# ClickHouse/libhdfs3

Hardware: AMD Instinct MI355X
Metric: device-resident CRC32C GiB/s over 512 B HDFS chunks; % of HBM roofline (higher is better)
Workload: dtype u8

## Files before the change

libhdfs3_amd/csrc/client/block_reader.cpp:

```cpp
#include "hdfs3_client.h"

#include <hip/hip_runtime.h>
#include <sys/socket.h>
#include <sys/uio.h>
#include <time.h>

#include <algorithm>
#include <cerrno>
#include <chrono>
#include <condition_variable>
#include <cstdlib>
#include <cstring>
#include <deque>
#include <mutex>
#include <new>
#include <string>
#include <thread>
#include <vector>

#include "../copy_pool.h"
#include "../ctx.h"
#include "../numa.h"
#include "block_reader.h"
#include "hdfs3_crc.h"
#include "net.h"
#include "wire.h"

using namespace hdfs3crc;

namespace {

constexpr int kDefaultBatchPackets = 64;
constexpr int kDefaultTimeoutMs = 60000;
constexpr size_t kMaxResponse = 10u << 20;
constexpr int kSlots = 3;
constexpr int kPhases = 8;
constexpr int kWaitPollUs = 20;
std::atomic<uint64_t> g_phase_ns[kPhases] = {};

uint64_t thread_cpu_ns() {
    timespec ts{};
    clock_gettime(CLOCK_THREAD_CPUTIME_ID, &ts);
    return uint64_t(ts.tv_sec) * 1000000000ull + uint64_t(ts.tv_nsec);
}
constexpr int kMaxSlots = 64;
constexpr int32_t kMaxPacketData = 16 << 20;
constexpr size_t kArenaCacheMax = 6;
constexpr size_t kPacketGuess = 64 * 1024 + 512 + 16;

struct PacketRef {
    uint64_t data_off, crc_off;
    uint32_t data_len;
    uint32_t skip;
    uint32_t deliver;
};

struct Batch {
    PacketArena a;
    size_t used = 0;
    std::vector<PacketRef> pk;
    bool verified = false;
    int64_t bad_pkt = -1;
    size_t dpkt = 0, doff = 0;
    bool dense = false, sealed = false;
    uint64_t d0 = 0, words_used = 0, data_used = 0;
    std::vector<uint64_t> chunk0;
    bool uploaded = false;

    void reset() {
        used = 0;
        pk.clear();
        verified = false;
        bad_pkt = -1;
        dpkt = doff = 0;
        dense = sealed = false;
        d0 = words_used = data_used = 0;
        chunk0.clear();
        uploaded = false;
    }
};

bool dense_bpc(uint32_t bpc) { return round_bpc(bpc) || pieces_bpc(bpc); }

bool wire_layout_forced() {
    static const bool f = [] {
        const char *e = getenv("HDFS3_READER_LAYOUT");
        return e && std::strcmp(e, "wire") == 0;
    }();
    return f;
}

uint64_t now_ns() {
    return uint64_t(std::chrono::duration_cast<std::chrono::nanoseconds>(
                        std::chrono::steady_clock::now().time_since_epoch()).count());
}

struct Timer {
    std::atomic<uint64_t> &acc;
    uint64_t t0 = now_ns();
    explicit Timer(std::atomic<uint64_t> &a) : acc(a) {}
    ~Timer() { acc.fetch_add(now_ns() - t0, std::memory_order_relaxed); }
};

thread_local bool t_hip_fault = false;

#if HDFS3_LAB
std::atomic<int> g_fail_prefetch_arenas{0};
#endif

int hip_err(hipError_t e, const char *what) {
    t_hip_fault = true;
    return fail(e == hipErrorOutOfMemory ? -ENOMEM : -EIO, "%s: %s", what, hipGetErrorString(e));
}

#define HIP_OK(expr)                                      \
    do {                                                  \
        hipError_t e_ = (expr);                           \
        if (e_ != hipSuccess) return hip_err(e_, #expr);  \
    } while (0)

int grow(PacketArena &a, size_t cap, size_t descs) {
    if (cap > a.cap) {
        if (a.h) (void)hipHostFree(a.h);
        if (a.d) (void)hipFree(a.d);
        a.h = a.d = nullptr;
        a.cap = 0;
        HIP_OK(hipHostMalloc(reinterpret_cast<void **>(&a.h), cap, pinned_host_flags()));
        HIP_OK(hipMalloc(reinterpret_cast<void **>(&a.d), cap));
        a.cap = cap;
    }
    if (descs > a.desc_cap) {
        if (a.h_desc) (void)hipHostFree(a.h_desc);
        if (a.d_desc) (void)hipFree(a.d_desc);
        a.h_desc = a.d_desc = nullptr;
        a.desc_cap = 0;
        HIP_OK(hipHostMalloc(reinterpret_cast<void **>(&a.h_desc), descs * sizeof(DevSegment), pinned_host_flags()));
        HIP_OK(hipMalloc(reinterpret_cast<void **>(&a.d_desc), descs * sizeof(DevSegment)));
        a.desc_cap = descs;
    }
    if (!a.d_res) {
        HIP_OK(hipMalloc(reinterpret_cast<void **>(&a.d_res), sizeof(unsigned long long)));
        HIP_OK(hipHostMalloc(reinterpret_cast<void **>(&a.h_res), sizeof(unsigned long long), pinned_host_flags()));
        HIP_OK(hipEventCreateWithFlags(&a.done, hipEventDisableTiming | hipEventBlockingSync));
    }
    return 0;
}

}

struct hdfs3_block_reader {
    int fd = -1;
    int timeout_ms = kDefaultTimeoutMs;
    int batch_packets = kDefaultBatchPackets;
    bool verify = true;
    hdfs3_crc_ctx *ctx = nullptr;
    bool own_ctx = true;
    bool prefetch = false;
    wire::ExtendedBlock block;
    int64_t start = 0, end_offset = 0;
    uint32_t chunk_size = 0;
    uint32_t checksum_size = 0;
    const uint32_t *tables = nullptr;

    int64_t recv_cursor = 0;
    int64_t last_seqno = -1;
    bool range_done = false;
    bool trailer_ok = false;
    std::atomic<bool> local_fault{false};
    bool have_pending_hdr = false;
    wire::PacketHeader pending_hdr;
    bool header_ahead = true;
    bool have_next_raw = false;
    uint8_t next_raw[wire::kPacketHeaderSize];

    std::mutex mu;
    std::condition_variable cv;
    std::vector<Batch> slot;
    std::deque<int> ready;
    std::deque<int> free_slots;
    bool recv_done = false;
    int recv_error = 0;
    std::string recv_msg;
    bool stop = false;
    std::thread rx;

    int64_t delivered = 0;
    bool sent_status = false;
    int error = 0;
    std::string error_msg;

    std::atomic<uint64_t> packets{0}, batches{0};
    std::atomic<uint64_t> dev_launches{0}, dev_bytes{0};
    hipEvent_t dev_done = nullptr;
    std::atomic<uint64_t> t_ns[kPhases] = {};
    enum WaitMode { kWaitPoll, kWaitBlock, kWaitSpin } wait_mode = kWaitPoll;
    bool copy_nt = false;
    uint8_t *dest = nullptr;
    int64_t rx_out = 0;
    void eager(const uint8_t *src, int64_t useful) {
        if (dest && useful > 0 && rx_out + useful <= end_offset - start) std::memcpy(dest + rx_out, src, size_t(useful));
        rx_out += useful;
    }

    int sticky(int code, const std::string &msg) {
        error = code;
        error_msg = msg;
        return fail(code, "%s", msg.c_str());
    }

    int check_response() {
        std::string resp;
        if (int rc = net::read_delimited(fd, resp, kMaxResponse, timeout_ms))
            return sticky(rc, "RemoteBlockReader: failed to read BlockOpResponseProto");
        wire::BlockOpResponse r;
        if (!wire::decode_block_op_response(resp.data(), resp.size(), r))
            return sticky(-EPROTO, "RemoteBlockReader cannot parse BlockOpResponseProto from Datanode response");
        if (r.status != wire::kSuccess)
            return sticky(-EIO, "RemoteBlockReader: Datanode return an error when sending read request: " +
                                    (r.message.empty() ? std::string("check Datanode's log") : r.message));
        if (!r.has_checksum_info) return sticky(-EPROTO, "RemoteBlockReader: response lacks ReadOpChecksumInfoProto");
        chunk_size = r.bytes_per_checksum;
        switch (r.checksum_type) {
        case wire::kChecksumNull: verify = false; checksum_size = 0; break;
        case wire::kChecksumCrc32c: checksum_size = 4; tables = ctx->d_tables_by[0]; break;
        case wire::kChecksumCrc32: checksum_size = 4; tables = ctx->d_tables_by[1]; break;
        default: return sticky(-EPROTO, "RemoteBlockReader cannot recognize checksum type");
        }
        if (chunk_size == 0 || chunk_size > 0x7FFFFFFFu)
            return sticky(-EPROTO, "RemoteBlockReader invalid chunk size");
        const int64_t first = int64_t(r.chunk_offset);
        if (first < 0 || first > start || first <= start - int64_t(chunk_size))
            return sticky(-EPROTO, "RemoteBlockReader invalid first chunk offset");
        return 0;
    }

    int rx_fail(int code, const std::string &msg) {
        recv_msg = msg;
        return code;
    }

    int read_header(wire::PacketHeader &h) {
        if (have_pending_hdr) {
            h = pending_hdr;
            have_pending_hdr = false;
            return 0;
        }
        if (have_next_raw) {
            have_next_raw = false;
            if (!h.decode(next_raw, sizeof(next_raw))) return rx_fail(-EPROTO, "Invalid PacketHeader");
            return 0;
        }
        uint8_t buf[wire::kPacketHeaderSize];
        if (int rc = net::recv_fully(fd, buf, sizeof(buf)))
            return rx_fail(rc, "RemoteBlockReader: failed to read block header");
        if (!h.decode(buf, sizeof(buf))) return rx_fail(-EPROTO, "Invalid PacketHeader");
        return 0;
    }

    int receive(Batch &b) {
        Timer tm(t_ns[0]);
        b.reset();
        while (int(b.pk.size()) < batch_packets && !range_done) {
            wire::PacketHeader h;
            if (int rc = read_header(h)) return rc;
            if (!h.sanity_check(last_seqno)) return rx_fail(-EIO, "RemoteBlockReader: Packet failed on sanity check");
            if (h.data_len <= 0) {
                last_seqno = h.seqno;
                range_done = true;
                break;
            }
            if (h.data_len > kMaxPacketData) return rx_fail(-EIO, "Invalid Packet, dataLen exceeds 16 MiB");
            if (h.offset_in_block > recv_cursor || recv_cursor - h.offset_in_block >= h.data_len)
                return rx_fail(-EIO, "Invalid Packet, offsetInBlock does not continue the block");
            const uint64_t chunks = (uint64_t(h.data_len) + chunk_size - 1) / chunk_size;
            const uint64_t crc_len = chunks * checksum_size;
            if (int64_t(h.packet_len) != 4 + int64_t(h.data_len) + int64_t(crc_len))
                return rx_fail(-EIO, "Invalid Packet, packetLen does not match dataLen and checksums");
            const uint64_t size = crc_len + uint64_t(h.data_len);
            if (b.pk.empty())
                b.dense = verify && checksum_size == 4 && dense_bpc(chunk_size) && !wire_layout_forced();
            if (b.dense) {
                if (b.pk.empty()) {
                    const uint64_t exp_data = std::max<uint64_t>(uint64_t(h.data_len), uint64_t(64) << 10);
                    const uint64_t max_crc = (exp_data + chunk_size - 1) / chunk_size * checksum_size;
                    b.d0 = (uint64_t(batch_packets) * max_crc + 4095) & ~uint64_t(4095);
                    const uint64_t need = b.d0 + uint64_t(h.data_len);
                    if (need > b.a.cap)
                        if (int rc = grow(b.a, need, size_t(batch_packets))) return rx_fail(rc, "arena growth failed");
                } else if (b.sealed || b.words_used + crc_len > b.d0 ||
                           b.d0 + b.data_used + uint64_t(h.data_len) > b.a.cap) {
                    pending_hdr = h;
                    have_pending_hdr = true;
                    break;
                }
                iovec v[3] = {{b.a.h + b.words_used, crc_len}, {b.a.h + b.d0 + b.data_used, size_t(h.data_len)},
                              {next_raw, header_ahead ? sizeof(next_raw) : 0}};
                if (int rc = net::recv_fully_iov(fd, v, 3))
                    return rx_fail(rc, "RemoteBlockReader: failed to read packet payload");
                have_next_raw = header_ahead;
                last_seqno = h.seqno;
                packets.fetch_add(1, std::memory_order_relaxed);
                int64_t ahead = recv_cursor - h.offset_in_block;
                ahead = ahead > 0 ? ahead : 0;
                const int64_t useful =
                    std::max<int64_t>(0, std::min<int64_t>(h.data_len - ahead, end_offset - recv_cursor));
                b.pk.push_back(PacketRef{b.d0 + b.data_used, b.words_used, uint32_t(h.data_len), uint32_t(ahead),
                                         uint32_t(useful)});
                eager(b.a.h + b.d0 + b.data_used + ahead, useful);
                b.chunk0.push_back(b.words_used / 4);
                b.words_used += crc_len;
                b.data_used += uint64_t(h.data_len);
                b.used = b.d0 + b.data_used;
                if (h.data_len % chunk_size) b.sealed = true;
                const int64_t reached = recv_cursor + h.data_len - ahead;
                recv_cursor = reached;
                if (reached >= end_offset) {
                    if (int rc = read_trailer()) return rc;
                    range_done = true;
                }
                continue;
            }
            uint64_t off = ((b.used + crc_len + 15) & ~uint64_t(15)) - crc_len;
            if (off + size > b.a.cap) {
                if (!b.pk.empty()) {
                    pending_hdr = h;
                    have_pending_hdr = true;
                    break;
                }
                if (int rc = grow(b.a, size + 64, size_t(batch_packets))) return rx_fail(rc, "arena growth failed");
                off = ((crc_len + 15) & ~uint64_t(15)) - crc_len;
            }
            iovec v[2] = {{b.a.h + off, size}, {next_raw, header_ahead ? sizeof(next_raw) : 0}};
            if (int rc = net::recv_fully_iov(fd, v, 2))
                return rx_fail(rc, "RemoteBlockReader: failed to read packet payload");
            have_next_raw = header_ahead;
            last_seqno = h.seqno;
            packets.fetch_add(1, std::memory_order_relaxed);
            int64_t ahead = recv_cursor - h.offset_in_block;
            ahead = ahead > 0 ? ahead : 0;
            const int64_t useful = std::max<int64_t>(0, std::min<int64_t>(h.data_len - ahead, end_offset - recv_cursor));
            b.pk.push_back(PacketRef{off + crc_len, off, uint32_t(h.data_len), uint32_t(ahead), uint32_t(useful)});
            eager(b.a.h + off + crc_len + ahead, useful);
            b.used = off + size;
            const int64_t reached = recv_cursor + h.data_len - ahead;
            recv_cursor = reached;
            if (reached >= end_offset) {
                if (int rc = read_trailer()) return rc;
                range_done = true;
            }
        }
        return 0;
    }

    int read_trailer() {
        wire::PacketHeader t;
        if (int rc = read_header(t)) return rc;
        if (t.last_packet_in_block && t.data_len == 0) {
            last_seqno = t.seqno;
            trailer_ok = true;
        }
        return 0;
    }

    int launch(Batch &b) {
        Timer tm(t_ns[2]);
        batches.fetch_add(1, std::memory_order_relaxed);
        if (!verify) {
            b.verified = true;
            return 0;
        }
        LaunchEnv env = launch_env(ctx, &b.a.pieces);
        env.tables = tables;
        env.fold = ctx->d_fold_by[tables == ctx->d_tables_by[1]];
        HIP_OK(hipMemcpyAsync(b.a.d, b.a.h, b.used, hipMemcpyHostToDevice, ctx->stream));
        b.uploaded = true;
        HIP_OK(hipMemsetAsync(b.a.d_res, 0, sizeof(unsigned long long), ctx->stream));
        if (b.dense) {
            ChunkLaunch a{};
            a.data = b.a.d + b.d0;
            a.len = b.data_used;
            a.bpc = chunk_size;
            a.crc_be = b.a.d;
            a.result = b.a.d_res;
            a.check_short_tail = 0;
            HIP_OK(launch_chunks(env, a, true));
        } else {
            std::vector<DevPacket> hp(b.pk.size());
            for (size_t i = 0; i < b.pk.size(); ++i)
                hp[i] = DevPacket{b.pk[i].data_off, b.pk[i].crc_off, b.pk[i].data_len, 0};
            HIP_OK(launch_packet_batch(env, b.a.d, hp.data(), hp.size(), chunk_size, true, 0,
                                       b.a.d_res, b.a.h_desc, b.a.d_desc));
        }
        ++ctx->launches;
        HIP_OK(hipMemcpyAsync(b.a.h_res, b.a.d_res, sizeof(unsigned long long), hipMemcpyDeviceToHost, ctx->stream));
        HIP_OK(hipEventRecord(b.a.done, ctx->stream));
        return 0;
    }

    int acquire(Batch &b) {
        Timer tm(t_ns[1]);
#if HDFS3_LAB
        if (prefetch && g_fail_prefetch_arenas.load() > 0 && g_fail_prefetch_arenas.fetch_sub(1) > 0) {
            t_hip_fault = true;
            return rx_fail(fail(-ENOMEM, "injected pinned-memory shortage"), "arena allocation failed");
        }
#endif
        if (!b.a.h) {
            std::lock_guard<std::mutex> lk(ctx->arena_mu);
            if (!ctx->arena_cache.empty()) {
                b.a = ctx->arena_cache.back();
                ctx->arena_cache.pop_back();
            }
        }
        if (int rc = grow(b.a, std::max(b.a.cap, size_t(batch_packets) * kPacketGuess), size_t(batch_packets)))
            return rx_fail(rc, "arena allocation failed");
        return 0;
    }

    void receiver() {
        (void)hipSetDevice(ctx->device);
        bind_thread_to_device(ctx->device);
        const uint64_t cpu0 = thread_cpu_ns();
        struct CpuAdd {
            hdfs3_block_reader *r;
            uint64_t c0;
            ~CpuAdd() { r->t_ns[7].fetch_add(thread_cpu_ns() - c0, std::memory_order_relaxed); }
        } cpu_add{this, cpu0};
        for (;;) {
            int s;
            {
                Timer idle(t_ns[5]);
                std::unique_lock<std::mutex> lk(mu);
                cv.wait(lk, [&] { return stop || !free_slots.empty(); });
                if (stop) break;
                s = free_slots.front();
                free_slots.pop_front();
            }
            Batch &b = slot[s];
            t_hip_fault = false;
            int rc = acquire(b);
            if (!rc) rc = receive(b);
            if (!rc && !b.pk.empty()) {
                rc = launch(b);
                if (rc) recv_msg = hdfs3_crc_last_error();
            }
            if (rc && t_hip_fault) local_fault = true;
            {
                std::lock_guard<std::mutex> lk(mu);
                if (!rc && !b.pk.empty())
                    ready.push_back(s);
                else
                    free_slots.push_back(s);
                if (rc) recv_error = rc;
                if (rc || range_done) recv_done = true;
            }
            cv.notify_all();
            if (rc || range_done) break;
        }
    }

    void start_receiver() {
        for (int i = 0; i < int(slot.size()); ++i) free_slots.push_back(i);
        rx = std::thread([this] { receiver(); });
    }

    int wait_event(hipEvent_t ev) {
        Timer tm(t_ns[3]);
        if (wait_mode == kWaitBlock) {
            HIP_OK(hipEventSynchronize(ev));
        } else {
            for (;;) {
                const hipError_t q = hipEventQuery(ev);
                if (q == hipSuccess) break;
                if (q != hipErrorNotReady) HIP_OK(q);
                if (wait_mode == kWaitPoll) std::this_thread::sleep_for(std::chrono::microseconds(kWaitPollUs));
            }
        }
        return 0;
    }

    int wait(Batch &b) {
        if (b.verified) return 0;
        if (int rc = wait_event(b.a.done)) return rc;
        const unsigned long long r = *b.a.h_res;
        if (r && b.dense) {
            const uint64_t chunk = ~r;
            b.bad_pkt = int64_t(std::upper_bound(b.chunk0.begin(), b.chunk0.end(), chunk) - b.chunk0.begin()) - 1;
        } else if (r) {
            b.bad_pkt = int64_t((~r) >> 32);
        }
        b.verified = true;
        return 0;
    }

    void maybe_send_status() {
        if (sent_status || error || !trailer_ok) return;
        {
            std::lock_guard<std::mutex> lk(mu);
            if (!recv_done || recv_error || !ready.empty()) return;
        }
        const std::string msg = wire::encode_client_read_status(verify ? wire::kChecksumOk : wire::kSuccess);
        if (net::write_delimited(fd, msg, timeout_ms) == 0) sent_status = true;
    }

    int32_t read(uint8_t *out, int32_t len) {
        if (error) return fail(error, "%s", error_msg.c_str());
        if (len <= 0 || !out) return fail(-EINVAL, "invalid read buffer");
        int32_t total = 0;
        while (total < len) {
            int s;
            {
                Timer idle(t_ns[6]);
                std::unique_lock<std::mutex> lk(mu);
                cv.wait(lk, [&] { return !ready.empty() || recv_done; });
                if (ready.empty()) {
                    if (recv_error) {
                        const int code = recv_error;
                        const std::string msg = recv_msg;
                        lk.unlock();
                        if (total) {
                            error = code;
                            error_msg = msg;
                            return total;
                        }
                        return sticky(code, msg);
                    }
                    break;
                }
                s = ready.front();
            }
            Batch &b = slot[s];
            if (int rc = wait(b)) {
                local_fault = true;
                return total ? total : sticky(rc, hdfs3_crc_last_error());
            }
            const size_t limit = b.bad_pkt >= 0 ? size_t(b.bad_pkt) : b.pk.size();
            {
                Timer tm(t_ns[4]);
                while (total < len && b.dpkt < limit) {
                    const PacketRef &p = b.pk[b.dpkt];
                    const size_t avail = p.deliver - b.doff;
                    const size_t n = std::min<size_t>(avail, size_t(len - total));
                    if (dest && out + total == dest + delivered)
                        ;
                    else if (copy_nt && n >= 4096)
                        memcpy_stream(out + total, b.a.h + p.data_off + p.skip + b.doff, n);
                    else
                        std::memcpy(out + total, b.a.h + p.data_off + p.skip + b.doff, n);
                    total += int32_t(n);
                    b.doff += n;
                    delivered += int64_t(n);
                    if (b.doff == p.deliver) {
                        ++b.dpkt;
                        b.doff = 0;
                    }
                }
            }
            if (b.dpkt == limit) {
                if (b.bad_pkt >= 0) {
                    sticky(-EIO, "ChecksumException: RemoteBlockReader: checksum not match for Block: " +
                                     std::to_string(block.block_id) + " (packet " + std::to_string(b.bad_pkt) +
                                     " of a GPU batch)");
                    return total ? total : error;
                }
                {
                    std::lock_guard<std::mutex> lk(mu);
                    ready.pop_front();
                    free_slots.push_back(s);
                }
                cv.notify_all();
            }
        }
        maybe_send_status();
        return total;
    }

    int32_t read_dev(uint8_t *d_out, int32_t len) {
        if (error) return fail(error, "%s", error_msg.c_str());
        if (len <= 0 || !d_out) return fail(-EINVAL, "invalid read buffer");
        DeviceGuard guard(ctx->device);
        hipPointerAttribute_t at{};
        if (hipPointerGetAttributes(&at, d_out) != hipSuccess || at.type != hipMemoryTypeDevice ||
            at.device != ctx->device) {
            (void)hipGetLastError();
            return fail(-EINVAL, "read_dev: the buffer is not device memory of device %d", ctx->device);
        }
        if (!dev_done) HIP_OK(hipEventCreateWithFlags(&dev_done, hipEventDisableTiming | hipEventBlockingSync));
        int32_t total = 0;
        int failed = 0;
        bool enqueued = false;
        std::vector<CopyRange> rg;
        auto complete = [&]() -> int {
            if (!enqueued) return 0;
            HIP_OK(hipEventRecord(dev_done, ctx->stream));
            if (int rc = wait_event(dev_done)) return rc;
            enqueued = false;
            return 0;
        };
        while (total < len && !failed) {
            int s;
            {
                Timer idle(t_ns[6]);
                std::unique_lock<std::mutex> lk(mu);
                cv.wait(lk, [&] { return !ready.empty() || recv_done; });
                if (ready.empty()) {
                    if (recv_error) {
                        error = recv_error;
                        error_msg = recv_msg;
                        failed = error;
                    }
                    break;
                }
                s = ready.front();
            }
            Batch &b = slot[s];
            if (int rc = wait(b)) {
                local_fault = true;
                error = failed = rc;
                error_msg = hdfs3_crc_last_error();
                break;
            }
            const size_t limit = b.bad_pkt >= 0 ? size_t(b.bad_pkt) : b.pk.size();
            {
                Timer tm(t_ns[4]);
                rg.clear();
                const int32_t before = total;
                while (total < len && b.dpkt < limit) {
                    const PacketRef &p = b.pk[b.dpkt];
                    const size_t n = std::min<size_t>(p.deliver - b.doff, size_t(len - total));
                    rg.push_back(CopyRange{p.data_off + p.skip + b.doff, uint64_t(total), n});
                    total += int32_t(n);
                    b.doff += n;
                    delivered += int64_t(n);
                    if (b.doff == p.deliver) {
                        ++b.dpkt;
                        b.doff = 0;
                    }
                }
                int rc = 0;
                if (total > before) {
                    const bool own_upload = !b.uploaded;
                    if (own_upload) {
                        const hipError_t e = hipMemcpyAsync(b.a.d, b.a.h, b.used, hipMemcpyHostToDevice, ctx->stream);
                        if (e != hipSuccess) rc = hip_err(e, "hipMemcpyAsync");
                        b.uploaded = true;
                    }
                    unsigned launched = 0;
                    if (!rc) rc = gather_dev(ctx, d_out, size_t(len), b.a.d, b.used, rg.data(), rg.size(), &launched);
                    enqueued = true;
                    if (!rc && own_upload) rc = complete();
                    dev_launches.fetch_add(launched, std::memory_order_relaxed);
                    dev_bytes.fetch_add(uint64_t(total - before), std::memory_order_relaxed);
                }
                if (rc) {
                    local_fault = true;
                    error = failed = rc;
                    error_msg = hdfs3_crc_last_error();
                    break;
                }
            }
            if (b.dpkt == limit) {
                if (b.bad_pkt >= 0) {
                    failed = sticky(-EIO, "ChecksumException: RemoteBlockReader: checksum not match for Block: " +
                                              std::to_string(block.block_id) + " (packet " + std::to_string(b.bad_pkt) +
                                              " of a GPU batch)");
                    break;
                }
                {
                    std::lock_guard<std::mutex> lk(mu);
                    ready.pop_front();
                    free_slots.push_back(s);
                }
                cv.notify_all();
            }
        }
        if (int rc = complete()) {
            local_fault = true;
            error = failed = rc;
            error_msg = hdfs3_crc_last_error();
            total = 0;
        }
        if (failed) return total ? total : fail(error, "%s", error_msg.c_str());
        maybe_send_status();
        return total;
    }

    int64_t available() {
        std::lock_guard<std::mutex> lk(mu);
        int64_t a = 0;
        for (int s : ready) {
            const Batch &b = slot[s];
            if (!b.verified) continue;
            const size_t limit = b.bad_pkt >= 0 ? size_t(b.bad_pkt) : b.pk.size();
            for (size_t i = b.dpkt; i < limit; ++i) a += b.pk[i].deliver - (i == b.dpkt ? b.doff : 0);
        }
        return a;
    }

    ~hdfs3_block_reader() {
        if (rx.joinable()) {
            {
                std::lock_guard<std::mutex> lk(mu);
                stop = true;
            }
            cv.notify_all();
            if (fd >= 0) shutdown(fd, SHUT_RDWR);
            rx.join();
        }
        if (ctx) (void)hipStreamSynchronize(ctx->stream);
        if (dev_done) (void)hipEventDestroy(dev_done);
        for (int i = 0; i < kPhases; ++i) g_phase_ns[i].fetch_add(t_ns[i].load(), std::memory_order_relaxed);
        const size_t cache_max = std::max(kArenaCacheMax, slot.size());
        for (Batch &b : slot) {
            if (!b.a.h) continue;
            bool cached = false;
            if (ctx && !own_ctx) {
                std::lock_guard<std::mutex> lk(ctx->arena_mu);
                if (ctx->arena_cache.size() < cache_max) {
                    ctx->arena_cache.push_back(b.a);
                    cached = true;
                }
            }
            if (!cached) b.a.release();
            b.a = PacketArena();
        }
        if (ctx && own_ctx) ctx_release(ctx);
        net::close_fd(fd);
    }
};

namespace hdfs3crc {

bool block_reader_local_fault(const hdfs3_block_reader *r) { return r && r->local_fault.load(); }

int64_t block_reader_batch_bytes(const hdfs3_reader_opts *opts) {
    const int bp = opts && opts->batch_packets > 0 ? opts->batch_packets : kDefaultBatchPackets;
    return int64_t(bp) * 64 * 1024;
}

int64_t block_reader_arena_bytes(const hdfs3_reader_opts *opts) {
    const int bp = opts && opts->batch_packets > 0 ? opts->batch_packets : kDefaultBatchPackets;
    return int64_t(bp) * int64_t(kPacketGuess + sizeof(DevSegment)) + int64_t(sizeof(unsigned long long));
}

int open_block_reader(const char *host, int port, const hdfs3_block_id *blk, int64_t start, int64_t len,
                      const char *client_name, const hdfs3_reader_opts *opts, hdfs3_crc_ctx *shared_ctx,
                      hdfs3_block_reader **out, int slots, uint8_t *dest) {
    if (!out || !host || !blk || start < 0 || len < 0) return fail(-EINVAL, "invalid argument");
    *out = nullptr;
    hdfs3_block_reader *r = new (std::nothrow) hdfs3_block_reader();
    if (!r) return fail(-ENOMEM, "reader allocation");
    int nslots = slots > 0 ? slots : kSlots;
    if (const char *e = getenv("HDFS3_READER_SLOTS"); e && slots <= 0)
        nslots = std::atoi(e);
    r->slot.resize(size_t(std::min(std::max(nslots, kSlots), kMaxSlots)));
    r->prefetch = slots > 0;
    {
        const char *w = getenv("HDFS3_READER_WAIT");
        r->wait_mode = !w                            ? hdfs3_block_reader::kWaitPoll
                       : std::strcmp(w, "spin") == 0  ? hdfs3_block_reader::kWaitSpin
                       : std::strcmp(w, "block") == 0 ? hdfs3_block_reader::kWaitBlock
                                                      : hdfs3_block_reader::kWaitPoll;
        const char *ha = getenv("HDFS3_READER_HEADER_AHEAD");
        r->header_ahead = !(ha && ha[0] == '0');
#if HDFS3_COPY_NT_AVAILABLE
        const char *nt = getenv("HDFS3_READER_COPY_NT");
        r->copy_nt = nt && nt[0] == '1' && __builtin_cpu_supports("avx2");
#endif
    }
    const int device = opts ? opts->device : 0;
    r->verify = opts ? opts->verify != 0 : true;
    if (opts && opts->batch_packets > 0) r->batch_packets = opts->batch_packets;
    if (const char *bp = getenv("HDFS3_READER_BATCH_PACKETS")) {
        const int v = std::atoi(bp);
        if (v > 0 && v <= 1024) r->batch_packets = v;
    }
    if (opts && opts->timeout_ms > 0) r->timeout_ms = opts->timeout_ms;
    r->block.pool_id = blk->pool_id ? blk->pool_id : "";
    r->block.block_id = blk->block_id;
    r->block.generation_stamp = blk->generation_stamp;
    r->block.num_bytes = blk->num_bytes;
    r->start = r->recv_cursor = start;
    r->end_offset = start + len;
    r->dest = dest;
    if (shared_ctx) {
        r->ctx = shared_ctx;
        r->own_ctx = false;
    } else if (int rc = ctx_acquire(device, &r->ctx)) {
        delete r;
        return rc;
    }
    r->fd = net::connect_tcp(host, port, r->timeout_ms);
    if (r->fd < 0) {
        const int rc = r->fd;
        delete r;
        return fail(rc, "RemoteBlockReader: Failed to connect to %s:%d", host, port);
    }
    wire::ReadBlockRequest req;
    req.block = r->block;
    req.client_name = client_name ? client_name : "libhdfs3_amd";
    req.offset = uint64_t(start);
    req.len = uint64_t(len);
    const std::string frame = wire::encode_read_block(req);
    if (int rc = net::write_fully(r->fd, frame.data(), frame.size(), r->timeout_ms)) {
        delete r;
        return fail(rc, "DataTransferProtocolSender cannot send read request to datanode");
    }
    if (int rc = r->check_response()) {
        delete r;
        return rc;
    }
    if (int rc = net::set_recv_timeout(r->fd, r->timeout_ms)) {
        delete r;
        return fail(rc, "RemoteBlockReader: cannot set the socket's read timeout");
    }
    r->start_receiver();
    *out = r;
    return 0;
}

}

extern "C" {

int hdfs3_block_reader_open(const char *host, int port, const hdfs3_block_id *blk, int64_t start,
                            int64_t len, const char *client_name, const hdfs3_reader_opts *opts,
                            hdfs3_block_reader **out) {
    return open_block_reader(host, port, blk, start, len, client_name, opts, nullptr, out);
}

int32_t hdfs3_block_reader_read(hdfs3_block_reader *r, void *buf, int32_t len) {
    if (!r) return fail(-EINVAL, "null reader");
    return r->read(static_cast<uint8_t *>(buf), len);
}

int32_t hdfs3_block_reader_read_dev(hdfs3_block_reader *r, void *d_buf, int32_t len) {
    if (!r) return fail(-EINVAL, "null reader");
    return r->read_dev(static_cast<uint8_t *>(d_buf), len);
}

int hdfs3_block_reader_device_stats(hdfs3_block_reader *r, uint64_t *gather_launches, uint64_t *bytes_gathered) {
    if (!r) return fail(-EINVAL, "null reader");
    if (gather_launches) *gather_launches = r->dev_launches.load();
    if (bytes_gathered) *bytes_gathered = r->dev_bytes.load();
    return 0;
}

int64_t hdfs3_block_reader_available(hdfs3_block_reader *r) { return r ? r->available() : 0; }

int hdfs3_block_reader_stats(hdfs3_block_reader *r, uint32_t *bpc, uint64_t *packets, uint64_t *gpu_batches) {
    if (!r) return fail(-EINVAL, "null reader");
    if (bpc) *bpc = r->chunk_size;
    if (packets) *packets = r->packets.load();
    if (gpu_batches) *gpu_batches = r->batches.load();
    return 0;
}

#if HDFS3_LAB
void hdfs3x_fail_prefetch_arenas(int n) { g_fail_prefetch_arenas = n; }

int hdfs3x_block_reader_timing(hdfs3_block_reader *r, uint64_t *out5) {
    if (!r || !out5) return fail(-EINVAL, "invalid argument");
    for (int i = 0; i < 5; ++i) out5[i] = r->t_ns[i].load();
    return 0;
}
#endif

int hdfs3_block_reader_close(hdfs3_block_reader *r) {
    delete r;
    return 0;
}

int hdfs3_reader_phase_ns(uint64_t *out, int n, int reset) {
    if (!out || n < 0 || n > kPhases) return fail(-EINVAL, "invalid argument");
    for (int i = 0; i < n; ++i) out[i] = reset ? g_phase_ns[i].exchange(0) : g_phase_ns[i].load();
    if (reset)
        for (int i = n; i < kPhases; ++i) g_phase_ns[i].store(0);
    return 0;
}

}
```

libhdfs3_amd/csrc/client/input_stream.cpp:

```cpp
#include <algorithm>
#include <cerrno>
#include <cstdlib>
#include <cstring>
#include <deque>
#include <new>
#include <string>
#include <vector>

#include "../ctx.h"
#include "block_reader.h"
#include "hdfs3_client.h"
#include "hdfs3_crc.h"

using namespace hdfs3crc;

namespace {

constexpr int64_t kMaxSkip = 128 * 1024;
constexpr int kShallowArenas = 6;

struct Node {
    std::string host;
    int port;
    bool operator==(const Node &o) const { return port == o.port && host == o.host; }
};

struct Block {
    std::string pool;
    hdfs3_block_id id;
    int64_t offset, length;
    std::vector<Node> replicas;
};

struct Ahead {
    int block;
    hdfs3_block_reader *reader;
    hdfs3_crc_ctx *ctx;
    Node node;
};

int posix_fail(int err, const std::string &msg) {
    fail(-err, "%s", msg.c_str());
    errno = err;
    return -1;
}

}

struct hdfs3_input_stream {
    std::vector<Block> blocks;
    int64_t file_length = 0;
    hdfs3_reader_opts opts{0, 1, 0, 0};
    std::string client_name;
    hdfs3_crc_ctx *ctx = nullptr;
    int64_t cursor = 0;
    int64_t end_of_cur_block = 0;
    int cur = -1;
    hdfs3_block_reader *reader = nullptr;
    Node cur_node;
    std::vector<Node> failed;
    uint64_t failovers = 0, opened = 0;
    std::string last_error;
    int ahead_blocks = 0;
    int64_t ahead_bytes = 0;
    std::deque<Ahead> ahead;
    hdfs3_crc_ctx *reader_ctx = nullptr;
    uint64_t ahead_opened = 0;
    uint64_t ahead_faults = 0;

    ~hdfs3_input_stream() {
        drop_ahead(-1);
        drop_reader();
        if (ctx) ctx_release(ctx);
    }

    void drop_reader() {
        if (reader) hdfs3_block_reader_close(reader);
        reader = nullptr;
        if (reader_ctx) ctx_release(reader_ctx);
        reader_ctx = nullptr;
    }

    static void close_ahead(Ahead &a) {
        hdfs3_block_reader_close(a.reader);
        ctx_release(a.ctx);
    }

    void drop_ahead(int keep_from) {
        for (auto it = ahead.begin(); it != ahead.end();) {
            if (keep_from >= 0 && it->block > keep_from && it->block <= keep_from + ahead_blocks) {
                ++it;
                continue;
            }
            close_ahead(*it);
            it = ahead.erase(it);
        }
    }

    void schedule_ahead(int i) {
        for (auto it = ahead.begin(); it != ahead.end(); ++it) {
            if (it->block != i) continue;
            reader = it->reader;
            reader_ctx = it->ctx;
            cur_node = it->node;
            ahead.erase(it);
            break;
        }
        drop_ahead(i);
        if (ahead_blocks <= 0) return;
        const int64_t unit = block_reader_batch_bytes(&opts);
        for (int j = i + 1; j <= i + ahead_blocks && j < int(blocks.size()); ++j) {
            auto at = std::find_if(ahead.begin(), ahead.end(), [&](const Ahead &a) { return a.block >= j; });
            if (at != ahead.end() && at->block == j) continue;
            const Block &b = blocks[size_t(j)];
            if (b.length <= 0 || b.replicas.empty()) continue;
            const int64_t want = std::min<int64_t>(b.length, ahead_bytes > 0 ? ahead_bytes : b.length);
            const int64_t arena = block_reader_arena_bytes(&opts);
            const int64_t cap = int64_t(pool_pinned_cap_bytes());
            const int64_t fit = std::max<int64_t>(0, cap - int64_t(kShallowArenas) * arena) /
                                int64_t(ahead_blocks + 1) / arena;
            const int slots = int(std::max<int64_t>(3, std::min<int64_t>({(want + unit - 1) / unit + 1, 64, fit})));
            hdfs3_crc_ctx *c = nullptr;
            if (ctx_acquire(opts.device, &c, true)) break;
            hdfs3_block_id id = b.id;
            id.pool_id = b.pool.c_str();
            hdfs3_block_reader *r = nullptr;
            const Node &n = b.replicas.front();
            if (open_block_reader(n.host.c_str(), n.port, &id, 0, b.length, client_name.c_str(), &opts, c, &r,
                                  slots)) {
                ctx_release(c);
                continue;
            }
            ++ahead_opened;
            ahead.insert(at, Ahead{j, r, c, n});
        }
    }

    int find_block(int64_t pos) const {
        auto it = std::upper_bound(blocks.begin(), blocks.end(), pos,
                                   [](int64_t p, const Block &b) { return p < b.offset; });
        if (it == blocks.begin()) return -1;
        const int i = int(it - blocks.begin()) - 1;
        return pos < blocks[i].offset + blocks[i].length ? i : -1;
    }

    const Node *best_node(const Block &b) const {
        for (const Node &n : b.replicas)
            if (std::find(failed.begin(), failed.end(), n) == failed.end()) return &n;
        return nullptr;
    }

    int setup(const Block &b, int64_t start, int64_t len, hdfs3_block_reader **out, Node *node,
              uint8_t *dest = nullptr) {
        std::string why;
        for (;;) {
            const Node *n = best_node(b);
            if (!n) {
                last_error = "InputStreamImpl: all nodes have been tried and no valid replica can be read for Block: " +
                             std::to_string(b.id.block_id) + (why.empty() ? "" : " (last: " + why + ")");
                return -EIO;
            }
            hdfs3_block_id id = b.id;
            id.pool_id = b.pool.c_str();
            const int rc = open_block_reader(n->host.c_str(), n->port, &id, start, len, client_name.c_str(), &opts,
                                             ctx, out, 0, dest);
            if (rc == 0) {
                *node = *n;
                ++opened;
                return 0;
            }
            if (rc == -ENOTSUP || rc == -ENOMEM || rc == -ENODEV) {
                last_error = hdfs3_crc_last_error();
                return rc;
            }
            why = hdfs3_crc_last_error();
            failed.push_back(*n);
        }
    }

    void seek_to_block(int i) {
        drop_reader();
        cur = i;
        end_of_cur_block = blocks[i].offset + blocks[i].length;
        failed.clear();
        if ((ahead_blocks > 0 || !ahead.empty()) && cursor == blocks[i].offset) schedule_ahead(i);
        else if (!ahead.empty()) drop_ahead(i);
    }

    static int32_t reader_read(hdfs3_block_reader *r, uint8_t *buf, int32_t size, bool dev) {
        return dev ? hdfs3_block_reader_read_dev(r, buf, size) : hdfs3_block_reader_read(r, buf, size);
    }

    int32_t read_one_block(uint8_t *buf, int32_t size, bool dev) {
        const Block &b = blocks[cur];
        for (;;) {
            if (!reader) {
                const int64_t off = cursor - b.offset;
                if (int rc = setup(b, off, b.length - off, &reader, &cur_node)) return rc;
            }
            const int32_t todo = int32_t(std::min<int64_t>(size, end_of_cur_block - cursor));
            const int32_t n = reader_read(reader, buf, todo, dev);
            if (n > 0) {
                cursor += n;
                return n;
            }
            if (dev && n == -EINVAL) {
                last_error = hdfs3_crc_last_error();
                return n;
            }
            if (block_reader_local_fault(reader)) {
                last_error = hdfs3_crc_last_error();
                const bool prefetched = reader_ctx != nullptr;
                drop_reader();
                if (prefetched) {
                    ++ahead_faults;
                    continue;
                }
                return n < 0 ? n : -EIO;
            }
            ++failovers;
            failed.push_back(cur_node);
            drop_reader();
        }
    }

    int32_t read(uint8_t *buf, int32_t size, bool dev = false) {
        if (cursor >= file_length) return 0;
        if (cursor >= end_of_cur_block || cur < 0) {
            const int i = find_block(cursor);
            if (i < 0) return -EIO;
            seek_to_block(i);
        }
        return read_one_block(buf, size, dev);
    }

    int fetch_range(const Block &b, int64_t start, int64_t len, uint8_t *out, bool dev) {
        std::vector<Node> saved;
        saved.swap(failed);
        int rc = 0;
        for (;;) {
            hdfs3_block_reader *r = nullptr;
            Node node;
            const char *ev = getenv("HDFS3_READER_EAGER_COPY");
            const bool eager = !dev && !(ev && ev[0] == '0');
            if ((rc = setup(b, start, len, &r, &node, eager ? out : nullptr))) break;
            int64_t got = 0;
            int32_t n = 0;
            while (got < len) {
                n = reader_read(r, out + got, int32_t(std::min<int64_t>(len - got, 1 << 30)), dev);
                if (n <= 0) break;
                got += n;
            }
            const bool local = block_reader_local_fault(r);
            if (local) last_error = hdfs3_crc_last_error();
            hdfs3_block_reader_close(r);
            if (got == len) break;
            if (local || (dev && n == -EINVAL)) {
                if (!local) last_error = hdfs3_crc_last_error();
                rc = n < 0 ? n : -EIO;
                break;
            }
            ++failovers;
            failed.push_back(node);
        }
        failed.swap(saved);
        return rc;
    }

    int32_t pread(int64_t pos, uint8_t *buf, int32_t size, bool dev = false) {
        if (pos < 0 || pos >= file_length) return -EINVAL;
        const int32_t real = int32_t(std::min<int64_t>(size, file_length - pos));
        int64_t done = 0;
        while (done < real) {
            const int i = find_block(pos + done);
            if (i < 0) return -EIO;
            const Block &b = blocks[i];
            const int64_t start = pos + done - b.offset;
            const int64_t n = std::min<int64_t>(real - done, b.length - start);
            if (int rc = fetch_range(b, start, n, buf + done, dev)) return rc;
            done += n;
        }
        return real;
    }

    int seek(int64_t pos) {
        if (pos == cursor) return 0;
        if (pos > file_length) return -EOVERFLOW;
        if (reader && pos > cursor && pos < end_of_cur_block && pos - cursor <= kMaxSkip) {
            uint8_t scratch[16384];
            bool ok = true;
            while (cursor < pos) {
                const int32_t n = hdfs3_block_reader_read(reader, scratch, int32_t(std::min<int64_t>(sizeof(scratch), pos - cursor)));
                if (n <= 0) {
                    ok = false;
                    break;
                }
                cursor += n;
            }
            if (ok) return 0;
        }
        drop_reader();
        end_of_cur_block = 0;
        cursor = pos;
        return 0;
    }
};

extern "C" {

int hdfs3_input_open(const hdfs3_located_block *blocks, int n_blocks, const char *client_name,
                     const hdfs3_reader_opts *opts, hdfs3_input_stream **out) {
    if (!out || n_blocks < 0 || (n_blocks && !blocks)) return fail(-EINVAL, "invalid argument");
    *out = nullptr;
    hdfs3_input_stream *s = new (std::nothrow) hdfs3_input_stream();
    if (!s) return fail(-ENOMEM, "input stream allocation");
    if (opts) s->opts = *opts;
    s->client_name = client_name ? client_name : "libhdfs3_amd";
    int64_t expect = n_blocks ? blocks[0].offset : 0;
    for (int i = 0; i < n_blocks; ++i) {
        const hdfs3_located_block &lb = blocks[i];
        if (lb.offset != expect || int64_t(lb.block.num_bytes) < 0 || lb.n_replicas < 0 ||
            (lb.n_replicas && !lb.replicas)) {
            delete s;
            return fail(-EINVAL, "located block %d is not contiguous with its predecessor or malformed", i);
        }
        Block b;
        b.pool = lb.block.pool_id ? lb.block.pool_id : "";
        b.id = lb.block;
        b.id.pool_id = nullptr;
        b.offset = lb.offset;
        b.length = int64_t(lb.block.num_bytes);
        for (int k = 0; k < lb.n_replicas; ++k) {
            if (!lb.replicas[k].host) {
                delete s;
                return fail(-EINVAL, "replica %d of block %d has no host", k, i);
            }
            b.replicas.push_back(Node{lb.replicas[k].host, lb.replicas[k].port});
        }
        expect += b.length;
        s->blocks.push_back(std::move(b));
    }
    if (n_blocks && blocks[0].offset != 0) {
        delete s;
        return fail(-EINVAL, "the first block must start at file offset 0");
    }
    s->file_length = expect;
    if (int rc = ctx_acquire(s->opts.device, &s->ctx)) {
        delete s;
        return rc;
    }
    *out = s;
    return 0;
}

int32_t hdfs3_input_read(hdfs3_input_stream *s, void *buf, int32_t len) {
    if (!s || !buf || len <= 0) return posix_fail(EINVAL, "hdfsRead: invalid argument");
    s->last_error.clear();
    const int32_t rc = s->read(static_cast<uint8_t *>(buf), len);
    if (rc < 0) return posix_fail(-rc, s->last_error.empty() ? hdfs3_crc_last_error() : s->last_error);
    return rc;
}

int32_t hdfs3_input_pread(hdfs3_input_stream *s, int64_t pos, void *buf, int32_t len) {
    if (!s || !buf || len <= 0 || pos < 0) return posix_fail(EINVAL, "hdfsPread: invalid argument");
    s->last_error.clear();
    const int32_t rc = s->pread(pos, static_cast<uint8_t *>(buf), len);
    if (rc == -EINVAL) return posix_fail(EINVAL, "hdfsPread: position outside the file");
    if (rc < 0) return posix_fail(-rc, s->last_error.empty() ? hdfs3_crc_last_error() : s->last_error);
    return rc;
}

int32_t hdfs3_input_read_dev(hdfs3_input_stream *s, void *d_buf, int32_t len) {
    if (!s || !d_buf || len <= 0) return posix_fail(EINVAL, "hdfs3_input_read_dev: invalid argument");
    s->last_error.clear();
    const int32_t rc = s->read(static_cast<uint8_t *>(d_buf), len, true);
    if (rc < 0) return posix_fail(-rc, s->last_error.empty() ? hdfs3_crc_last_error() : s->last_error);
    return rc;
}

int32_t hdfs3_input_pread_dev(hdfs3_input_stream *s, int64_t pos, void *d_buf, int32_t len) {
    if (!s || !d_buf || len <= 0 || pos < 0) return posix_fail(EINVAL, "hdfs3_input_pread_dev: invalid argument");
    if (pos >= s->file_length) return posix_fail(EINVAL, "hdfs3_input_pread_dev: position outside the file");
    s->last_error.clear();
    const int32_t rc = s->pread(pos, static_cast<uint8_t *>(d_buf), len, true);
    if (rc < 0) return posix_fail(-rc, s->last_error.empty() ? hdfs3_crc_last_error() : s->last_error);
    return rc;
}

int hdfs3_input_seek(hdfs3_input_stream *s, int64_t pos) {
    if (!s || pos < 0) return posix_fail(EINVAL, "hdfsSeek: invalid argument");
    if (int rc = s->seek(pos))
        return posix_fail(-rc, "InputStreamImpl: seek over EOF, seek target: " + std::to_string(pos));
    return 0;
}

int64_t hdfs3_input_tell(hdfs3_input_stream *s) {
    if (!s) return posix_fail(EINVAL, "hdfsTell: invalid argument");
    return s->cursor;
}

int hdfs3_input_available(hdfs3_input_stream *s) {
    if (!s) return posix_fail(EINVAL, "hdfsAvailable: invalid argument");
    const int64_t a = s->reader ? hdfs3_block_reader_available(s->reader) : 0;
    return int(std::min<int64_t>(a, 0x7FFFFFFF));
}

int64_t hdfs3_input_length(hdfs3_input_stream *s) { return s ? s->file_length : -1; }

int hdfs3_input_stats(hdfs3_input_stream *s, uint64_t *failovers, uint64_t *readers_opened) {
    if (!s) return fail(-EINVAL, "null stream");
    if (failovers) *failovers = s->failovers;
    if (readers_opened) *readers_opened = s->opened;
    return 0;
}

int hdfs3_input_set_readahead(hdfs3_input_stream *s, int blocks, int64_t max_bytes_per_block) {
    if (!s || blocks < 0 || max_bytes_per_block < 0) return fail(-EINVAL, "invalid argument");
    if (blocks > HDFS3_READAHEAD_MAX_BLOCKS)
        return fail(-EINVAL, "read-ahead of %d blocks: at most %d", blocks, HDFS3_READAHEAD_MAX_BLOCKS);
    s->ahead_blocks = blocks;
    s->ahead_bytes = max_bytes_per_block;
    if (blocks == 0) s->drop_ahead(-1);
    return 0;
}

int hdfs3_input_readahead_stats(hdfs3_input_stream *s, uint64_t *prefetch_readers_opened,
                                uint64_t *prefetch_local_faults) {
    if (!s) return fail(-EINVAL, "null stream");
    if (prefetch_readers_opened) *prefetch_readers_opened = s->ahead_opened;
    if (prefetch_local_faults) *prefetch_local_faults = s->ahead_faults;
    return 0;
}

int hdfs3_input_close(hdfs3_input_stream *s) {
    delete s;
    return 0;
}

}
```

Baseline: 6103.

## Post caller read buffers so receiver thread copies packets directly into them

Adds a PostedWindow through which a blocked read() registers its output buffer, so the receive thread copies payload straight into that buffer as packets arrive. Delivery then skips the copy for bytes already placed, overlapping the copy with network receive. On failure it zeroes any partially written range. This brings mutex handoff and generation tracking between the threads, plus memset cleanup on error paths. It is enabled by default only for non-verifying, non-prefetch readers without a dest, so it likely does not touch the device CRC benchmark path.

```diff
diff --git a/libhdfs3_amd/csrc/client/block_reader.cpp b/libhdfs3_amd/csrc/client/block_reader.cpp
--- a/libhdfs3_amd/csrc/client/block_reader.cpp
+++ b/libhdfs3_amd/csrc/client/block_reader.cpp
@@ -24,6 +24,7 @@
 #include "block_reader.h"
 #include "hdfs3_crc.h"
 #include "net.h"
+#include "posted_window.h"
 #include "wire.h"
 
 using namespace hdfs3crc;
@@ -53,6 +54,7 @@
     uint32_t data_len;
     uint32_t skip;
     uint32_t deliver;
+    PostedWindow::Placed placed{};
 };
 
 struct Batch {
@@ -196,10 +198,15 @@
     enum WaitMode { kWaitPoll, kWaitBlock, kWaitSpin } wait_mode = kWaitPoll;
     bool copy_nt = false;
     uint8_t *dest = nullptr;
+    bool post_reads = false;
+    PostedWindow win;
+    uint64_t live_gen = 0;
     int64_t rx_out = 0;
-    void eager(const uint8_t *src, int64_t useful) {
-        if (dest && useful > 0 && rx_out + useful <= end_offset - start) std::memcpy(dest + rx_out, src, size_t(useful));
+    PostedWindow::Placed eager(const uint8_t *src, int64_t useful) {
+        PostedWindow::Placed p{};
+        if (useful > 0) p = win.place(src, rx_out, useful);
         rx_out += useful;
+        return p;
     }
 
     int sticky(int code, const std::string &msg) {
@@ -306,7 +313,7 @@
                     std::max<int64_t>(0, std::min<int64_t>(h.data_len - ahead, end_offset - recv_cursor));
                 b.pk.push_back(PacketRef{b.d0 + b.data_used, b.words_used, uint32_t(h.data_len), uint32_t(ahead),
                                          uint32_t(useful)});
-                eager(b.a.h + b.d0 + b.data_used + ahead, useful);
+                b.pk.back().placed = eager(b.a.h + b.d0 + b.data_used + ahead, useful);
                 b.chunk0.push_back(b.words_used / 4);
                 b.words_used += crc_len;
                 b.data_used += uint64_t(h.data_len);
@@ -340,7 +347,7 @@
             ahead = ahead > 0 ? ahead : 0;
             const int64_t useful = std::max<int64_t>(0, std::min<int64_t>(h.data_len - ahead, end_offset - recv_cursor));
             b.pk.push_back(PacketRef{off + crc_len, off, uint32_t(h.data_len), uint32_t(ahead), uint32_t(useful)});
-            eager(b.a.h + off + crc_len + ahead, useful);
+            b.pk.back().placed = eager(b.a.h + off + crc_len + ahead, useful);
             b.used = off + size;
             const int64_t reached = recv_cursor + h.data_len - ahead;
             recv_cursor = reached;
@@ -503,15 +510,35 @@
         if (net::write_delimited(fd, msg, timeout_ms) == 0) sent_status = true;
     }
 
+    void end_call(uint8_t *out, int32_t good, bool posted, bool failed) {
+        if (!live_gen || !(posted || failed)) return;
+        const PostedWindow::Extent e = win.withdraw();
+        live_gen = 0;
+        uint8_t *base = posted ? out : dest;
+        const int64_t from = std::max<int64_t>(e.lo, posted ? int64_t(good) : delivered);
+        if (e.hi > from) std::memset(base + from, 0, size_t(e.hi - from));
+    }
+
     int32_t read(uint8_t *out, int32_t len) {
         if (error) return fail(error, "%s", error_msg.c_str());
         if (len <= 0 || !out) return fail(-EINVAL, "invalid read buffer");
+        bool posted = false;
+        const int32_t n = read_loop(out, len, posted);
+        end_call(out, std::max(n, 0), posted, n < 0 || error || local_fault.load());
+        return n;
+    }
+
+    int32_t read_loop(uint8_t *out, int32_t len, bool &posted) {
         int32_t total = 0;
         while (total < len) {
             int s;
             {
                 Timer idle(t_ns[6]);
                 std::unique_lock<std::mutex> lk(mu);
+                if (post_reads && !posted && ready.empty() && !recv_done) {
+                    live_gen = win.post(out, len, delivered - total);
+                    posted = true;
+                }
                 cv.wait(lk, [&] { return !ready.empty() || recv_done; });
                 if (ready.empty()) {
                     if (recv_error) {
@@ -540,8 +567,13 @@
                 while (total < len && b.dpkt < limit) {
                     const PacketRef &p = b.pk[b.dpkt];
                     const size_t avail = p.deliver - b.doff;
-                    const size_t n = std::min<size_t>(avail, size_t(len - total));
-                    if (dest && out + total == dest + delivered)
+                    size_t n = std::min<size_t>(avail, size_t(len - total));
+                    const PostedWindow::Placed &pl = p.placed;
+                    const bool live = pl.n > 0 && pl.gen == live_gen;
+                    const size_t lo = live ? size_t(pl.skip) : 0, hi = live ? size_t(pl.skip + pl.n) : 0;
+                    if (b.doff < lo) n = std::min(n, lo - b.doff);
+                    else if (b.doff < hi) n = std::min(n, hi - b.doff);
+                    if (b.doff >= lo && b.doff < hi && pl.at + (b.doff - lo) == out + total)
                         ;
                     else if (copy_nt && n >= 4096)
                         memcpy_stream(out + total, b.a.h + p.data_off + p.skip + b.doff, n);
@@ -707,6 +739,7 @@
             if (fd >= 0) shutdown(fd, SHUT_RDWR);
             rx.join();
         }
+        end_call(nullptr, 0, false, true);
         if (ctx) (void)hipStreamSynchronize(ctx->stream);
         if (dev_done) (void)hipEventDestroy(dev_done);
         for (int i = 0; i < kPhases; ++i) g_phase_ns[i].fetch_add(t_ns[i].load(), std::memory_order_relaxed);
@@ -783,6 +816,7 @@
     r->start = r->recv_cursor = start;
     r->end_offset = start + len;
     r->dest = dest;
+    if (dest && len > 0) r->live_gen = r->win.post(dest, len, 0);
     if (shared_ctx) {
         r->ctx = shared_ctx;
         r->own_ctx = false;
@@ -810,6 +844,10 @@
         delete r;
         return rc;
     }
+    if (!dest && !r->prefetch) {
+        const char *ev = getenv("HDFS3_READER_EAGER_COPY");
+        r->post_reads = ev && (ev[0] == '0' || ev[0] == '1') ? ev[0] == '1' : !r->verify;
+    }
     if (int rc = net::set_recv_timeout(r->fd, r->timeout_ms)) {
         delete r;
         return fail(rc, "RemoteBlockReader: cannot set the socket's read timeout");
diff --git a/libhdfs3_amd/csrc/client/input_stream.cpp b/libhdfs3_amd/csrc/client/input_stream.cpp
--- a/libhdfs3_amd/csrc/client/input_stream.cpp
+++ b/libhdfs3_amd/csrc/client/input_stream.cpp
@@ -238,6 +238,7 @@
         std::vector<Node> saved;
         saved.swap(failed);
         int rc = 0;
+        int64_t most = 0;
         for (;;) {
             hdfs3_block_reader *r = nullptr;
             Node node;
@@ -255,6 +256,7 @@
             if (local) last_error = hdfs3_crc_last_error();
             hdfs3_block_reader_close(r);
             if (got == len) break;
+            most = std::max(most, got);
             if (local || (dev && n == -EINVAL)) {
                 if (!local) last_error = hdfs3_crc_last_error();
                 rc = n < 0 ? n : -EIO;
@@ -264,6 +266,7 @@
             failed.push_back(node);
         }
         failed.swap(saved);
+        if (rc && !dev && most > 0) std::memset(out, 0, size_t(most));
         return rc;
     }
 
diff --git a/libhdfs3_amd/csrc/client/posted_window.h b/libhdfs3_amd/csrc/client/posted_window.h
--- /dev/null
+++ b/libhdfs3_amd/csrc/client/posted_window.h
@@ -0,0 +1,77 @@
+#pragma once
+
+#include <algorithm>
+#include <atomic>
+#include <condition_variable>
+#include <cstdint>
+#include <cstring>
+#include <mutex>
+
+namespace hdfs3crc {
+
+class PostedWindow {
+public:
+    struct Placed {
+        uint8_t *at = nullptr;
+        int64_t skip = 0;
+        int64_t n = 0;
+        uint64_t gen = 0;
+    };
+    struct Extent {
+        int64_t lo = 0, hi = 0;
+    };
+
+    uint64_t post(uint8_t *out, int64_t len, int64_t off) {
+        std::unique_lock<std::mutex> lk(m_);
+        cv_.wait(lk, [&] { return !busy_; });
+        out_ = out;
+        len_ = len;
+        off_ = off;
+        lo_ = len;
+        hi_ = 0;
+        armed_.store(out != nullptr && len > 0, std::memory_order_release);
+        return ++gen_;
+    }
+
+    Placed place(const uint8_t *src, int64_t off, int64_t n) {
+        if (!armed_.load(std::memory_order_acquire) || n <= 0) return Placed{};
+        std::unique_lock<std::mutex> lk(m_);
+        if (!armed_.load(std::memory_order_relaxed)) return Placed{};
+        const int64_t a = std::max(off, off_), b = std::min(off + n, off_ + len_);
+        if (b <= a) return Placed{};
+        Placed p{out_ + (a - off_), a - off, b - a, gen_};
+        lo_ = std::min(lo_, a - off_);
+        hi_ = std::max(hi_, b - off_);
+        busy_ = true;
+        lk.unlock();
+        std::memcpy(p.at, src + p.skip, size_t(p.n));
+        lk.lock();
+        busy_ = false;
+        lk.unlock();
+        cv_.notify_all();
+        return p;
+    }
+
+    Extent withdraw() {
+        std::unique_lock<std::mutex> lk(m_);
+        armed_.store(false, std::memory_order_release);
+        cv_.wait(lk, [&] { return !busy_; });
+        const Extent e{lo_, hi_};
+        out_ = nullptr;
+        len_ = off_ = 0;
+        lo_ = hi_ = 0;
+        return e;
+    }
+
+private:
+    std::mutex m_;
+    std::condition_variable cv_;
+    std::atomic<bool> armed_{false};
+    uint8_t *out_ = nullptr;
+    int64_t len_ = 0, off_ = 0;
+    int64_t lo_ = 0, hi_ = 0;
+    uint64_t gen_ = 0;
+    bool busy_ = false;
+};
+
+}
```

Result: slower. 5995 (-1.8%).
